# scverse/muon

Measured on AMD Instinct MI355X. Metric: cells/sec for TF-IDF+LSI(k=50), higher is better.
Workload: dtype f32

## Files before the change

include/muon_amd.h:

```cpp
#ifndef MUON_AMD_H
#define MUON_AMD_H

#include <stddef.h>
#include <stdint.h>

#ifdef __cplusplus
extern "C" {
#endif

typedef enum {
  MU_OK = 0,
  MU_ERR_ARG = -1,
  MU_ERR_HIP = -2,
  MU_ERR_NO_DEVICE = -3,
  MU_ERR_UNSUPPORTED = -4
} mu_status;

#define MU_DTYPE_F32 0
#define MU_DTYPE_F64 1

#define MU_TFIDF_LOG_TF 1
#define MU_TFIDF_LOG_IDF 2
#define MU_TFIDF_LOG_TFIDF 4

int mu_version(void);
const char* mu_last_error(void);
int mu_device_count(int* count);
int mu_set_device(int device);
int mu_device_info(int device, char* name, int len, int* n_cu, size_t* total_mem);
int mu_malloc(void** d_ptr, size_t bytes);
int mu_free(void* d_ptr);
int mu_memcpy_h2d(void* d_dst, const void* h_src, size_t bytes, void* stream);
int mu_memcpy_d2h(void* h_dst, const void* d_src, size_t bytes, void* stream);
int mu_memset(void* d_dst, int value, size_t bytes, void* stream);
int mu_stream_sync(void* stream);
int mu_host_hash64(const void* h_ptr, size_t n_bytes, int n_threads, uint64_t seed, uint64_t* h_out);

size_t mu_csr_row_col_sums_worksize(int64_t n_rows, int64_t n_cols);

int mu_csr_row_col_sums(int dtype, int64_t n_rows, int64_t n_cols, const int64_t* d_indptr,
                        const int32_t* d_indices, const void* d_values, double* d_rowsum,
                        double* d_colsum, void* d_work, size_t work_bytes, void* stream);

int mu_tfidf_idf(int dtype, int64_t n_cols, double n_obs, const double* d_colsum, int flags,
                 void* d_idf, void* stream);

int mu_tfidf_scale(int dtype, int64_t n_rows, const int64_t* d_indptr, const int32_t* d_indices,
                   const void* d_values, const double* d_rowsum, const void* d_idf, double scale,
                   int flags, void* d_out, unsigned long long* d_zero_count, void* stream);

int mu_tfidf_scale_sweep(int dtype, int64_t n_rows, int64_t n_cols, const int64_t* d_indptr,
                         const int32_t* d_indices, const void* d_values, const double* d_rowsum,
                         const void* d_idf, double scale, int flags, void* d_out,
                         unsigned long long* d_zero_count, void* d_work, size_t work_bytes,
                         int have_slab_ptr, void* stream);

int mu_csr_count_nonzero(int dtype, int64_t n_rows, const int64_t* d_indptr, const void* d_values,
                         int64_t* d_row_nnz, void* stream);
int mu_csr_compact_nonzero(int dtype, int64_t n_rows, const int64_t* d_indptr,
                           const int32_t* d_indices, const void* d_values,
                           const int64_t* d_new_indptr, int32_t* d_new_indices, void* d_new_values,
                           void* stream);
int mu_exclusive_scan_i64(int64_t n, const int64_t* d_in, int64_t* d_out, void* stream);

int mu_binarize_values(int dtype, int64_t nnz, void* d_values, void* stream);

size_t mu_csr_qc_worksize(int64_t n_rows, int64_t n_cols);
int mu_csr_qc(int dtype, int64_t n_rows, int64_t n_cols, const int64_t* d_indptr, const int32_t* d_indices,
              const void* d_values, int64_t* d_row_nnz, double* d_rowsum, int64_t* d_col_nnz, double* d_colsum,
              void* d_work, size_t work_bytes, const int64_t* d_slab_ptr, void* stream);

int mu_csr_submatrix_count(int64_t n_rows, int64_t n_cols, int64_t n_keep, const int64_t* d_indptr,
                           const int32_t* d_indices, const int64_t* d_rows, const int32_t* d_col_table,
                           int64_t* d_new_row_nnz, void* stream);
int mu_csr_submatrix_fill(int dtype, int64_t n_rows, int64_t n_cols, int64_t n_keep, const int64_t* d_indptr,
                          const int32_t* d_indices, const void* d_values, const int64_t* d_rows,
                          const int32_t* d_col_table, const int64_t* d_new_indptr, int32_t* d_new_indices,
                          void* d_new_values, void* stream);

int mu_frag_chunk(void);
int mu_frag_ranges(int64_t n_win, int64_t n_contigs, const int32_t* d_wchrom, const int32_t* d_wlo,
                   const int32_t* d_whi, const int64_t* d_chrom_ptr, const int32_t* d_start, int64_t max_len,
                   int64_t* d_rng_lo, int64_t* d_rng_len, void* stream);
int mu_frag_overlap_count(int64_t n_win, int64_t n_chunks, const int64_t* d_chunk_ptr, const int64_t* d_rng_lo,
                          const int64_t* d_rng_len, const int32_t* d_wlo, const int32_t* d_whi, const int32_t* d_start,
                          const int32_t* d_end, const int32_t* d_barcode, const int32_t* d_cell_of, int64_t n_barcodes,
                          int64_t n_obs, int64_t* d_chunk_cnt, void* stream);
int mu_frag_overlap_emit(int64_t n_win, int64_t n_chunks, const int64_t* d_chunk_ptr, const int64_t* d_rng_lo,
                         const int64_t* d_rng_len, const int32_t* d_wlo, const int32_t* d_whi, const int32_t* d_start,
                         const int32_t* d_end, const int32_t* d_barcode, const int32_t* d_score,
                         const int32_t* d_cell_of, int64_t n_barcodes, int64_t n_obs, int64_t n_features,
                         const int64_t* d_chunk_off, int64_t* d_keys, int32_t* d_vals, void* stream);
int mu_frag_pileup(int64_t n_win, int64_t n_chunks, const int64_t* d_chunk_ptr, const int64_t* d_rng_lo,
                   const int64_t* d_rng_len, const int32_t* d_wlo, const int32_t* d_whi, const int32_t* d_start,
                   const int32_t* d_end, const int32_t* d_barcode, const int32_t* d_score, const int32_t* d_cell_of,
                   int64_t n_barcodes, int64_t n_obs, int64_t width, int32_t* d_diff, void* stream);
int mu_frag_pileup_scan(int64_t n_obs, int64_t width, int64_t flank_size, int64_t center_dist, int32_t* d_diff,
                        int64_t* d_sums, void* stream);
int mu_frag_length_classes(int64_t n_take, const int32_t* d_start, const int32_t* d_end, const int32_t* d_barcode,
                           const int32_t* d_cell_of, int64_t n_barcodes, int64_t n_obs, int free_bound, int mono_bound,
                           int32_t* d_classes, void* stream);

size_t mu_csr_transpose_worksize(int64_t n_rows, int64_t n_cols, int64_t nnz);
int mu_csr_transpose(int dtype, int64_t n_rows, int64_t n_cols, int64_t nnz,
                     const int64_t* d_indptr, const int32_t* d_indices, const void* d_values,
                     int64_t* d_t_indptr, int32_t* d_t_indices, void* d_t_values, void* d_work,
                     size_t work_bytes, void* stream);

int mu_spmm_f32(int64_t n_rows, int64_t n_cols, const int64_t* d_indptr, const int32_t* d_indices,
                const float* d_values, const float* d_Q, int B, float* d_Y, int accumulate,
                void* stream);


int mu_spmm_stream_k(int64_t n_rows);

int mu_tfidf_scale_sweep_stream(int64_t n_rows, int64_t n_cols, const int64_t* d_indptr, const int32_t* d_indices,
                                const float* d_values, const double* d_rowsum, const float* d_idf, double scale,
                                int flags, float* d_out, unsigned long long* d_zero_count, void* d_work,
                                size_t work_bytes, int have_slab_ptr, const int64_t* d_slab_ptr,
                                const int64_t* d_row_dst, void* d_ent, void* stream);
int mu_csr_slab_ptr(int64_t n_rows, int64_t n_cols, const int64_t* d_indptr, const int32_t* d_indices, int64_t* d_sp,
                    void* stream);
int mu_csr_slab_ptr_width(int64_t n_rows, int64_t n_cols, int64_t width, const int64_t* d_indptr,
                          const int32_t* d_indices, int64_t* d_sp, void* stream);
int mu_csr_row_col_sums_sp(int dtype, int64_t n_rows, int64_t n_cols, const int64_t* d_indptr,
                           const int32_t* d_indices, const void* d_values, double* d_rowsum, double* d_colsum,
                           void* d_work, size_t work_bytes, const int64_t* d_slab_ptr, void* stream);
int mu_tfidf_scale_sweep_sp(int dtype, int64_t n_rows, int64_t n_cols, const int64_t* d_indptr,
                            const int32_t* d_indices, const void* d_values, const double* d_rowsum, const void* d_idf,
                            double scale, int flags, void* d_out, unsigned long long* d_zero_count,
                            const int64_t* d_slab_ptr, void* stream);
int mu_tpack4_supported(int64_t n_rows, int64_t n_cols, int64_t nnz);
int mu_tpack4_geometry(int64_t n_rows, int64_t n_cols, int64_t nnz, int64_t* rows_per_block, int* n_blocks,
                       int* tile_cols);
size_t mu_tpack4_worksize(int64_t n_rows, int64_t n_cols, int64_t nnz);
int mu_tpack4_count(int64_t n_rows, int64_t n_cols, int64_t nnz, const int64_t* d_indptr, const int32_t* d_indices,
                    int64_t* d_col_nnz, void* d_work, size_t work_bytes, const int64_t* d_slab_ptr, void* stream);
int mu_tpack4_fill_stream(int64_t n_rows, int64_t n_cols, int64_t nnz, const int64_t* d_indptr,
                          const int32_t* d_indices, const float* d_values, const int64_t* d_x_row_dst,
                          const void* d_x_ent, const int64_t* d_sptr, const int32_t* d_inv, void* d_ent, void* d_work,
                          size_t work_bytes, void* stream);
int mu_tpack4_fill_csr(int64_t n_rows, int64_t n_cols, int64_t nnz, const int64_t* d_indptr, const int32_t* d_indices,
                       const float* d_values, const int64_t* d_x_row_dst, const void* d_x_ent,
                       const int64_t* d_t_indptr, int32_t* d_t_indices, float* d_t_values, void* d_work,
                       size_t work_bytes, void* stream);
int mu_tpack4_status(const void* d_work, int64_t n_rows, int64_t n_cols, int64_t nnz, int* h_err);
size_t mu_tpack4_err_offset(int64_t n_rows, int64_t n_cols, int64_t nnz);
size_t mu_tpack4_cnt_offset(int64_t n_rows, int64_t n_cols, int64_t nnz);
int mu_tpack4_phase_cycles(unsigned long long* h_out6, int reset);
int mu_tperm_stage_pairs(void);
int mu_tperm_plan(int64_t n_rows, int64_t n_cols, int64_t nnz, const int64_t* d_indptr, const int32_t* d_indices,
                  const int64_t* d_x_row_dst, int tile_cols, const int64_t* d_tile_off, int32_t* d_ntile,
                  int32_t* d_tiles, uint32_t* d_cont, uint16_t* d_slots, void* stream);
int mu_tperm_fill(int64_t n_rows, int64_t n_cols, int64_t nnz, const int64_t* d_indptr, const int64_t* d_x_row_dst,
                  const void* d_x_ent, const int64_t* d_cdst, const void* d_cnt, const int64_t* d_tile_off,
                  const int32_t* d_tiles, const uint32_t* d_cont, const uint16_t* d_slots, void* d_ent, void* stream);
int mu_csr_stream_len(int64_t n_pos, const int32_t* d_perm, const int64_t* d_indptr, int64_t* d_len,
                      void* stream);
int mu_csr_stream_fill(int64_t n_pos, const int32_t* d_perm, const int64_t* d_indptr,
                       const int32_t* d_indices, const float* d_values, const int64_t* d_sptr,
                       void* d_ent, void* stream);
int mu_spmm_stream_f32(int64_t n_pos, int64_t n_cols, const int64_t* d_sptr, const void* d_ent,
                       const int32_t* d_perm, int k_layout, const float* d_Q, int B, float* d_Y,
                       void* stream);
int mu_csr_slice_stream(int n_ranges, const int64_t* h_row0, const int64_t* h_rows, const int64_t* h_lo,
                        const int64_t* h_hi, int64_t n_cols, const int64_t* d_indptr, const int32_t* d_indices,
                        const float* d_values, const int64_t* d_slab_ptr, int64_t* d_sptr, void* d_ent, uint32_t* d_rel,
                        void* stream);
int mu_spmm_stream_ranges_f32(int64_t n_pos, const int64_t* d_sptr, const void* d_ent, const int32_t* d_perm,
                              int k_layout, const float* d_Q, int64_t q_rows, float* d_Y, int64_t y_stride,
                              const uint32_t* d_tbl, int64_t tbl_stride, int n_ranges, const int32_t* h_ranges5,
                              int per_wg, void* stream);
int mu_spmm_stream_f64(int64_t n_pos, int64_t n_cols, const int64_t* d_sptr, const void* d_ent,
                       const int32_t* d_perm, int k_layout, const double* d_Q, int B, double* d_Y,
                       int accumulate, void* stream);
int mu_spmm_stream_slab_ok(int B, int K, int slab_cols);
int mu_spmm_stream_slab_f32(int64_t n_pos, int64_t n_cols, const int64_t* d_sptr, const void* d_ent,
                            const int32_t* d_perm, int k_layout, const float* d_Q, int B, float* d_Y,
                            int slab_cols, void* stream);
int mu_spmm_stream_ranges_slab_f32(int64_t n_pos, const int64_t* d_sptr, const void* d_ent, const int32_t* d_perm,
                                   int k_layout, const float* d_Q, int64_t q_rows, float* d_Y, int64_t y_stride,
                                   const uint32_t* d_tbl, int64_t tbl_stride, int n_ranges, const int32_t* h_ranges5,
                                   int per_wg, int slab_cols, void* stream);


int mu_spmm_ell16_waves(int64_t n_rows);
int mu_spmm_ell16_f32(int waves, int64_t n_pos, int64_t n_cols, const int32_t* d_hdr, const int64_t* d_wave_base,
                      const void* d_ent, const int32_t* d_perm, const float* d_Q, float* d_Y, void* stream);
int mu_spmm_ell16_f64(int waves, int64_t n_pos, int64_t n_cols, const int32_t* d_hdr, const int64_t* d_wave_base,
                      const void* d_ent, const int32_t* d_perm, const double* d_Q, double* d_Y, int accumulate,
                      void* stream);
int mu_spmm_ell16_parts(int64_t n_rows, int64_t n_cols, int wide, int* waves, int* parts);
int mu_spmm_ell16_parts_f32(int waves, int parts, int64_t n_pos, int64_t n_cols, const int32_t* d_hdr,
                            const int64_t* d_wave_base, const void* d_ent, const int32_t* d_perm, const float* d_Q,
                            float* d_Y, int64_t y_stride, void* stream);
int mu_spmm_ell16_parts_f64(int waves, int parts, int64_t n_pos, int64_t n_cols, const int32_t* d_hdr,
                            const int64_t* d_wave_base, const void* d_ent, const int32_t* d_perm, const double* d_Q,
                            double* d_Y, int64_t y_stride, void* stream);

int mu_ell16_fill(int64_t n_groups, int64_t n_cols, int64_t nnz, int slab_cols, const int32_t* d_indices, const float* d_values,
                  const int64_t* d_slab_ptr, const int32_t* d_perm, const int32_t* d_hdr, const int64_t* d_win_base,
                  void* d_ent, void* stream);


int mu_tune_set(const char* key, int value);
int mu_tune_get(const char* key);

int mu_spmm_f64(int64_t n_rows, int64_t n_cols, const int64_t* d_indptr, const int32_t* d_indices,
                const double* d_values, const double* d_Q, int B, double* d_Y, int accumulate,
                void* stream);

size_t mu_gram_worksize(int64_t n_rows, int B);
int mu_gram_f32(int64_t n_rows, int B, const float* d_A, double* d_G, double* d_colsum,
                void* d_work, size_t work_bytes, void* stream);

int mu_gram_cross_f32(int64_t n_rows, int B, const float* d_A, const float* d_Bm, double* d_C,
                      void* d_work, size_t work_bytes, void* stream);

int mu_dense_apply_f32(int64_t n_rows, int B, const float* d_A, const float* d_M,
                       const float* d_bias, float* d_Out, void* stream);
int mu_dense_project_out_f32(int64_t n_rows, int B, const float* d_A, const double* d_C, float* d_Z,
                             void* stream);

int mu_chol_rinv_f64(int B, int w, const double* d_G, float* d_M, int* d_flag, void* stream);

int mu_randn_f32(int64_t count, uint64_t seed, float* d_out, void* stream);

size_t mu_skinny_tn_worksize(int dtype, int64_t n_rows, int64_t D);
int mu_skinny_nn(int dtype, int64_t n_rows, int64_t D, int64_t ldY, const void* d_Y, const void* d_T,
                 void* d_out, void* stream);
int mu_skinny_tn(int dtype, int64_t n_rows, int64_t D, int64_t ldY, const void* d_Y, const void* d_Z,
                 void* d_C, void* d_work, size_t work_bytes, void* stream);
int mu_skinny_nn_f64_f32(int64_t n_rows, int64_t D, int64_t ldY, const float* d_Y, const double* d_T, double* d_out,
                         void* stream);
int mu_skinny_tn_f64_f32(int64_t n_rows, int64_t D, int64_t ldY, const float* d_Y, const double* d_Z, double* d_C,
                         void* d_work, size_t work_bytes, void* stream);

int mu_mofa_update_w(int dtype, int64_t D, int K, int G, const void* d_B, const void* d_tau,
                     const void* d_Gz, const void* d_Z2, const void* d_alpha, const void* d_lth,
                     const void* d_l1mth, int spikeslab, void* d_EW, void* d_EW2, void* d_gamma,
                     void* d_EWh2, void* d_sig2, void* stream);
int mu_mofa_update_z(int dtype, int64_t N, int K, int M, int G, const void* d_A, const void* d_pres,
                     const int32_t* d_grp, const void* d_Gw, const void* d_dw2, const void* d_alphaz,
                     const void* d_corr, void* d_EZ, void* d_EZ2, void* d_sig2, void* stream);

size_t mu_mofa_rowstats_work_doubles(int K);
int mu_mofa_rowstats(int dtype, int64_t r0, int64_t r1, int K, const void* d_E, const void* d_E2,
                     const void* d_wgt, const void* d_aux, int scale_out, void* d_out_pad, int ld, int col0,
                     void* d_out_t, int64_t ld_t, void* d_gram, void* d_s2, void* d_s1, double* d_work,
                     void* stream);

int mu_dense_col_moments_chunks(int64_t n_rows, int64_t D);
int mu_dense_col_moments(int dtype, int64_t r0, int64_t r1, int64_t D, const void* d_Y, int chunks,
                         double* d_partial, void* stream);

int mu_knn_filter_f64(int64_t n_q, int64_t c_lo, int64_t c_hi, int p_pad, const double* d_Xq, const double* d_Xc,
                      const double* d_sqq, const double* d_sqc, const double* d_thr, const int32_t* d_self_pos,
                      int cap, int32_t* d_buf_pos, double* d_buf_d, int32_t* d_cnt, void* stream);
int mu_knn_merge_f64(int64_t n_q, int kc, int cap, const double* d_cur_d, const int64_t* d_cur_p, const double* d_buf_d,
                     const int32_t* d_buf_pos, const int32_t* d_cnt, double* d_out_d, int64_t* d_out_p, double* d_thr,
                     void* stream);

int mu_wnn_bandwidth_f64(int64_t n, int p, const double* d_X, const int64_t* d_g_indptr, const int32_t* d_g_indices,
                         const int64_t* d_r_indptr, const int32_t* d_r_indices, int n_bw, double bbox,
                         double* d_csigma, int32_t* d_overflow, void* stream);

int mu_mofa_gs_update(int dtype, int64_t n, int K, const void* d_T, const void* d_b, const double* d_prior,
                      const double* d_lth, const double* d_l1mth, int spikeslab, void* d_E, void* d_E2,
                      void* d_gamma, void* d_Eh2, void* d_sig2, void* stream);

int mu_umap_strengths_f64(int64_t n, int k, const double* d_dist, const int64_t* d_idx, double target, double mean_all,
                          double* d_val, void* stream);

int mu_csr_densify_rows(int dtype, int64_t r0, int64_t r1, int64_t D, const int64_t* d_indptr,
                        const int32_t* d_indices, const void* d_values, void* d_out, void* stream);

int mu_mofa_jaakkola(int dtype, int64_t n, const void* d_zeta, const void* d_a, const void* d_b, void* d_out,
                     void* stream);

int mu_mofa_poisson_pseudo(int dtype, int64_t n_rows, int64_t D, int mode, const void* d_zeta, const void* d_Y,
                           const void* d_kappa, void* d_out, void* stream);

int64_t mu_mofa_poisson_blocks(int64_t n_own, int64_t n_other);
int64_t mu_mofa_poisson_blocks_for(int dtype, int mode, int K, int64_t n_own, int64_t n_other);
int mu_mofa_poisson_dense(int dtype, int mode, int64_t n_own, int64_t n_other, int K, int64_t other_block,
                          const void* d_E_own, const void* d_E_other, const void* d_kappa, void* d_part, void* stream);
int mu_mofa_poisson_sparse(int dtype, int mode, int64_t n_own, int K, const int64_t* d_indptr, const int32_t* d_indices,
                           const void* d_values, const void* d_E_own, const void* d_E_other, void* d_out, void* stream);
int mu_mofa_poisson_dense_ld(int dtype, int mode, int64_t n_own, int64_t n_other, int K, int ld, int64_t other_block,
                             const void* d_E_own, const void* d_E_other, const void* d_kappa, void* d_part,
                             void* stream);
int mu_mofa_poisson_sparse_ld(int dtype, int mode, int64_t n_own, int K, int ld, const int64_t* d_indptr,
                              const int32_t* d_indices, const void* d_values, const void* d_E_own, const void* d_E_other,
                              void* d_out, void* stream);

int mu_mofa_jaakkola_cols(int K);
int mu_mofa_pack_moments(int dtype, int64_t n, int K, int ldm, const void* d_E, const void* d_E2, void* d_M,
                         void* stream);
int64_t mu_mofa_jaakkola_blocks(int dtype, int K, int64_t n_own, int64_t n_other);
int mu_mofa_jaakkola_sweep(int dtype, int64_t n_own, int64_t n_other, int K, int64_t other_block, const void* d_E_own,
                           const void* d_E2_own, const void* d_E_other, const void* d_E2_other, const void* d_M_other,
                           int ldm, void* d_part, void* stream);

size_t mu_mofa_elbo_work_doubles(int K);
int mu_mofa_tau_elbo(int dtype, int64_t D, int K, int G, const void* d_yy, const void* d_Ngm,
                     const void* d_EW, const void* d_EW2, const void* d_B, const void* d_Gz,
                     const void* d_Z2, double a0, double b0, void* d_tau, void* d_ltau, double* d_elbo,
                     double* d_work, void* stream);
int mu_mofa_stats_resid(int dtype, int64_t D, int K, int64_t q_rows, const double* d_yy, const void* d_EW,
// ... 88 lines not shown
```

muon_amd/csrc/runtime.hip:

```cpp
#include <atomic>
#include <cstdarg>
#include <cstdio>
#include <cstring>
#include <thread>
#include <vector>
#include "common.hpp"

static thread_local char g_err[512] = "";

void mu_set_error(const char* fmt, ...) {
  va_list ap;
  va_start(ap, fmt);
  vsnprintf(g_err, sizeof(g_err), fmt, ap);
  va_end(ap);
}

int mu_num_cus() {
  static int cached[64] = {0};
  int dev = 0;
  if (hipGetDevice(&dev) != hipSuccess || dev < 0 || dev >= 64) return 256;
  if (cached[dev] == 0) {
    int n = 0;
    if (hipDeviceGetAttribute(&n, hipDeviceAttributeMultiprocessorCount, dev) != hipSuccess ||
        n <= 0)
      n = 256;
    cached[dev] = n;
  }
  return cached[dev];
}

static const char* const kTuneKeys[] = {"spmm_k", "spmm_mode", "gram_wg", "pack_wg", "tpack_dbg", "spmm_narrow_off", "ell_mode", "tfidf_wide", "tfidf_pipe", "nn_interleave", "tfidf_abl", "tfidf_sum_m", "tn_pipe", "nn_fast_off", "stream_pipe", "tpack4_m", "tpack4_c", "scale_stream_off", "tpack4_plain", "tpack4_abl", "tpack4_late", "tpack4_circ", "tpack4_off", "tperm_off", "pois_valu", "pois_lane", "spmm_slab"};
constexpr int kTuneN = sizeof(kTuneKeys) / sizeof(kTuneKeys[0]);
static int g_tune[kTuneN] = {};

extern "C" {

int mu_version(void) { return 807; }

int mu_tune_set(const char* key, int value) {
  MU_REQUIRE(key, "null key");
  for (int i = 0; i < kTuneN; ++i)
    if (strcmp(key, kTuneKeys[i]) == 0) {
      MU_REQUIRE(value >= 0, "negative value");
      MU_REQUIRE(i != 0 || value <= 16, "spmm_k must be 0..16");
      g_tune[i] = value;
      return MU_OK;
    }
  mu_set_error("mu_tune_set: unknown key %s", key);
  return MU_ERR_ARG;
}

int mu_tune_get(const char* key) {
  if (key)
    for (int i = 0; i < kTuneN; ++i)
      if (strcmp(key, kTuneKeys[i]) == 0) return g_tune[i];
  return -1;
}

const char* mu_last_error(void) { return g_err; }

int mu_device_count(int* count) {
  MU_REQUIRE(count, "null count");
  int n = 0;
  hipError_t e = hipGetDeviceCount(&n);
  if (e != hipSuccess) {
    *count = 0;
    mu_set_error("hipGetDeviceCount: %s", hipGetErrorString(e));
    return MU_ERR_NO_DEVICE;
  }
  *count = n;
  return MU_OK;
}

int mu_set_device(int device) {
  MU_CHECK_HIP(hipSetDevice(device));
  return MU_OK;
}

int mu_device_info(int device, char* name, int len, int* n_cu, size_t* total_mem) {
  hipDeviceProp_t p;
  MU_CHECK_HIP(hipGetDeviceProperties(&p, device));
  if (name && len > 0) {
    snprintf(name, (size_t)len, "%s (%s)", p.name, p.gcnArchName);
  }
  if (n_cu) *n_cu = p.multiProcessorCount;
  if (total_mem) *total_mem = p.totalGlobalMem;
  return MU_OK;
}

int mu_malloc(void** d_ptr, size_t bytes) {
  MU_REQUIRE(d_ptr, "null out pointer");
  MU_CHECK_HIP(hipMalloc(d_ptr, bytes));
  return MU_OK;
}

int mu_free(void* d_ptr) {
  MU_CHECK_HIP(hipFree(d_ptr));
  return MU_OK;
}

int mu_memcpy_h2d(void* d_dst, const void* h_src, size_t bytes, void* stream) {
  MU_CHECK_HIP(hipMemcpyAsync(d_dst, h_src, bytes, hipMemcpyHostToDevice, (hipStream_t)stream));
  return MU_OK;
}

int mu_memcpy_d2h(void* h_dst, const void* d_src, size_t bytes, void* stream) {
  MU_CHECK_HIP(hipMemcpyAsync(h_dst, d_src, bytes, hipMemcpyDeviceToHost, (hipStream_t)stream));
  return MU_OK;
}

int mu_memset(void* d_dst, int value, size_t bytes, void* stream) {
  MU_CHECK_HIP(hipMemsetAsync(d_dst, value, bytes, (hipStream_t)stream));
  return MU_OK;
}

static inline uint64_t mu_rotl64(uint64_t x, int r) { return (x << r) | (x >> (64 - r)); }
static const uint64_t kP1 = 0x9E3779B185EBCA87ull, kP2 = 0xC2B2AE3D27D4EB4Full, kP3 = 0x165667B19E3779F9ull,
                      kP4 = 0x85EBCA77C2B2AE63ull, kP5 = 0x27D4EB2F165667C5ull;
static inline uint64_t mu_round64(uint64_t acc, uint64_t in) { return mu_rotl64(acc + in * kP2, 31) * kP1; }
static inline uint64_t mu_avalanche64(uint64_t h) {
  h ^= h >> 33; h *= kP2; h ^= h >> 29; h *= kP3; h ^= h >> 32;
  return h;
}
static uint64_t mu_chunk_digest(const unsigned char* p, size_t n, uint64_t seed) {
  uint64_t v1 = seed + kP1 + kP2, v2 = seed + kP2, v3 = seed, v4 = seed - kP1;
  size_t i = 0;
  for (; i + 32 <= n; i += 32) {
    uint64_t w[4];
    memcpy(w, p + i, 32);
    v1 = mu_round64(v1, w[0]); v2 = mu_round64(v2, w[1]); v3 = mu_round64(v3, w[2]); v4 = mu_round64(v4, w[3]);
  }
  uint64_t h = mu_rotl64(v1, 1) + mu_rotl64(v2, 7) + mu_rotl64(v3, 12) + mu_rotl64(v4, 18);
  h = (h ^ mu_round64(0, v1)) * kP1 + kP4; h = (h ^ mu_round64(0, v2)) * kP1 + kP4;
  h = (h ^ mu_round64(0, v3)) * kP1 + kP4; h = (h ^ mu_round64(0, v4)) * kP1 + kP4;
  h += (uint64_t)n;
  for (; i + 8 <= n; i += 8) {
    uint64_t w;
    memcpy(&w, p + i, 8);
    h = mu_rotl64(h ^ mu_round64(0, w), 27) * kP1 + kP4;
  }
  for (; i < n; ++i) h = mu_rotl64(h ^ (p[i] * kP5), 11) * kP1;
  return mu_avalanche64(h);
}

int mu_host_hash64(const void* h_ptr, size_t n_bytes, int n_threads, uint64_t seed, uint64_t* h_out) {
  MU_REQUIRE(h_out && (h_ptr || n_bytes == 0), "null pointer");
  const size_t chunk = (size_t)16 << 20;
  const size_t n_chunks = n_bytes ? (n_bytes + chunk - 1) / chunk : 1;
  std::vector<uint64_t> dig(n_chunks, 0);
  const unsigned char* p = (const unsigned char*)h_ptr;
  std::atomic<size_t> next(0);
  auto work = [&]() {
    for (;;) {
      const size_t c = next.fetch_add(1);
      if (c >= n_chunks) break;
      const size_t lo = c * chunk, hi = (lo + chunk < n_bytes) ? lo + chunk : n_bytes;
      dig[c] = mu_chunk_digest(p + lo, hi - lo, seed + c);
    }
  };
  int T = n_threads < 1 ? 1 : (n_threads > 64 ? 64 : n_threads);
  if ((size_t)T > n_chunks) T = (int)n_chunks;
  std::vector<std::thread> th;
  try {
    if (T > 1) {
      th.reserve(T - 1);
      for (int t = 1; t < T; ++t) th.emplace_back(work);
    }
  } catch (...) {
  }
  work();
  for (auto& x : th) x.join();
  uint64_t h = seed ^ kP5 ^ (uint64_t)n_bytes;
  for (size_t c = 0; c < n_chunks; ++c) h = mu_rotl64(h ^ mu_round64(0, dig[c]), 27) * kP1 + kP4;
  *h_out = mu_avalanche64(h);
  return MU_OK;
}

int mu_stream_sync(void* stream) {
  MU_CHECK_HIP(hipStreamSynchronize((hipStream_t)stream));
  return MU_OK;
}

}
```

muon_amd/csrc/tperm.hip:

```cpp
#include <type_traits>
#include <utility>

#include "common.hpp"
#pragma clang diagnostic ignored "-Winline-asm"

namespace {

constexpr int kT = 1024, kNW = 16;
constexpr int kMaxC = 512;
constexpr int kCap = 9216;
constexpr int kH0 = 72;
constexpr int kW0 = 76;
constexpr int kS0 = 110;
constexpr int kSlotP = 16;
constexpr int kNone = 0xff;

#define MU_TP_CLOB                                                                                                      \
  "v72", "v73", "v74", "v75", "v76", "v77", "v78", "v79", "v80", "v81", "v82", "v83", "v84", "v85", "v86", "v87", "v88", \
      "v89", "v90", "v91", "v92", "v93", "v94", "v95", "v96", "v97", "v98", "v99", "v100", "v101", "v102", "v103",       \
      "v104", "v105", "v106", "v107", "v108", "v109", "v110", "v111", "v112", "v113", "v114", "v115", "v116", "v117",    \
      "v118", "v119", "v120", "v121", "v122", "v123", "v124", "v125", "v126", "v127"

template <int L>
__device__ __forceinline__ int tp_writelane_c(int v, int x) {
// ... 77 lines not shown
      const int ws = wave_sum_all(n);
      if (lane == 0 && ws) atomicAdd(&s_tot, (unsigned)ws);
      __syncthreads();
      total = s_tot;
      __syncthreads();
      if (total <= (unsigned)kCap) break;
      if (tid == 0) s_tot = 0u;
      int w = ((int)(cend - cb) / 2 / 16) * 16;
      w = w < 16 ? 16 : w;
      cend = (int)cb + w;
      __syncthreads();
    }
    if (REC) {
      if (tid == 0) tiles[tb + t] = (int32_t)cb;
      const unsigned over = (unsigned)__ballot(n > 32);
      if (lane == 0) {
        int pa = kNone, pb = kNone;
        if (over) {
          pa = __builtin_ctz(over);
          const unsigned o2 = over & (over - 1u);
          if (o2) pb = __builtin_ctz(o2);
        }
        cont[(tc + t) * kNW + wave] = (uint32_t)(pa | (pb << 8));
      }
      if (total > 0u) {
        const int W = cend - (int)cb;
        for (int k = 0; k < n; ++k) atomicOr(&bm[wave][indices[cur + k] - (int)cb], 1u << sub);
        __syncthreads();
        uint32_t mine = 0;
        if (tid < W)
          for (int w = 0; w < kNW; ++w) mine += (uint32_t)__popc(bm[w][tid]);
        uint32_t incl = mine;
#pragma unroll
        for (int off = 1; off < 64; off <<= 1) {
          const uint32_t u = __shfl_up(incl, off, 64);
          if (lane >= off) incl += u;
        }
        if (lane == 63) wsum[wave] = incl;
        __syncthreads();
        uint32_t run = incl - mine;
        for (int w = 0; w < wave; ++w) run += wsum[w];
        if (tid < W)
          for (int w = 0; w < kNW; ++w) {
            fs[w][tid] = run;
            run += (uint32_t)__popc(bm[w][tid]);
          }
        __syncthreads();
        for (int k = 0; k < n; ++k) {
          const int c = indices[cur + k] - (int)cb;
          slots[dst0 + cur + k] = (uint16_t)(fs[wave][c] + (uint32_t)__popc(bm[wave][c] & ((1u << sub) - 1u)));
        }
        __syncthreads();
        if (tid < W)
          for (int w = 0; w < kNW; ++w) bm[w][tid] = 0u;
      }
    }
    cur += n;
    cb = cend;
  }
  if (tid == 0) {
    if (REC) tiles[tb + t] = (int32_t)n_cols;
    else ntile[g] = t;
  }
}

template <int J>
__device__ __forceinline__ void tp_issue_circ(uint64_t b0, uint64_t b1, uint64_t tb0, uint64_t tb1, unsigned s0, unsigned s1,
                                              unsigned m0, unsigned m1, unsigned sub, unsigned sub8, unsigned sub8w,
                                              unsigned sub2, unsigned sub2w) {
  unsigned long long save;
  unsigned p0, p1, q0, q1;
  asm volatile(
      "s_mov_b64 %[save], exec\n\t"
      "v_cmp_gt_u32 vcc, %[s0], %[sub]\n\t"
      "v_cndmask_b32 %[p0], %[sub8], %[sub8w], vcc\n\t"
      "v_cndmask_b32 %[q0], %[sub2], %[sub2w], vcc\n\t"
      "v_cmp_gt_u32 vcc, %[s1], %[sub]\n\t"
      "v_cndmask_b32 %[p1], %[sub8], %[sub8w], vcc\n\t"
      "v_cndmask_b32 %[q1], %[sub2], %[sub2w], vcc\n\t"
      "s_mov_b32 exec_lo, %[m0]\n\t"
      "s_mov_b32 exec_hi, 0\n\t"
      "global_load_dwordx2 v[%c[C]:%c[V]], %[p0], %[b0]\n\t"
      "global_load_ushort v%c[S], %[q0], %[tb0]\n\t"
      "s_mov_b32 exec_lo, 0\n\t"
      "s_mov_b32 exec_hi, %[m1]\n\t"
      "global_load_dwordx2 v[%c[C]:%c[V]], %[p1], %[b1]\n\t"
      "global_load_ushort v%c[S], %[q1], %[tb1]\n\t"
      "s_mov_b64 exec, %[save]"
      : [save] "=&s"(save), [p0] "=&v"(p0), [p1] "=&v"(p1), [q0] "=&v"(q0), [q1] "=&v"(q1)
      : [sub] "v"(sub), [sub8] "v"(sub8), [sub8w] "v"(sub8w), [sub2] "v"(sub2), [sub2w] "v"(sub2w), [b0] "s"(b0),
        [b1] "s"(b1), [tb0] "s"(tb0), [tb1] "s"(tb1), [s0] "s"(s0), [s1] "s"(s1), [m0] "s"(m0), [m1] "s"(m1),
        [C] "i"(kW0 + 2 * J), [V] "i"(kW0 + 2 * J + 1), [S] "i"(kS0 + J)
      : MU_TP_CLOB, "vcc", "memory");
}
__device__ __forceinline__ void tp_issue_cont(uint64_t a0, uint64_t a1, uint64_t t0, uint64_t t1, int n0, int n1,
                                              unsigned sub8, unsigned sub2) {
  unsigned long long save, m0, m1;
  asm volatile(
      "s_bfm_b64 %[m0], %[n0], 0\n\t"
      "s_bfm_b64 %[m1], %[n1], 32\n\t"
      "s_mov_b64 %[save], exec\n\t"
      "v_mov_b32 v%c[C], 0x7fffffff\n\t"
      "s_mov_b64 exec, %[m0]\n\t"
      "global_load_dwordx2 v[%c[C]:%c[V]], %[o8], %[a0]\n\t"
      "global_load_ushort v%c[S], %[o2], %[t0]\n\t"
      "s_mov_b64 exec, %[m1]\n\t"
      "global_load_dwordx2 v[%c[C]:%c[V]], %[o8], %[a1]\n\t"
      "global_load_ushort v%c[S], %[o2], %[t1]\n\t"
      "s_mov_b64 exec, %[save]"
      : [save] "=&s"(save), [m0] "=&s"(m0), [m1] "=&s"(m1)
      : [o8] "v"(sub8), [o2] "v"(sub2), [a0] "s"(a0), [a1] "s"(a1), [t0] "s"(t0), [t1] "s"(t1), [n0] "s"(n0), [n1] "s"(n1),
        [C] "i"(kW0 + 2 * kSlotP), [V] "i"(kW0 + 2 * kSlotP + 1), [S] "i"(kS0 + kSlotP)
      : MU_TP_CLOB, "memory");
}
template <int J>
__device__ __forceinline__ void tp_pad_slot() {
  asm volatile("v_mov_b32 v%c0, 0x7fffffff" ::"i"(kW0 + 2 * J) : MU_TP_CLOB);
}
template <int J>
__device__ __forceinline__ void tp_retire_slot(int cend, int pad) {
  asm volatile(
      "v_cmp_le_i32 vcc, %0, v%c1\n\t"
      "v_cndmask_b32 v%c1, %2, v%c1, vcc" ::"s"(cend),
      "i"(kW0 + 2 * J), "v"(pad)
      : MU_TP_CLOB, "vcc");
}
__device__ __forceinline__ void tp_wait_all() { asm volatile("s_waitcnt vmcnt(0)" ::: MU_TP_CLOB, "memory"); }
template <int R>
__device__ __forceinline__ unsigned tp_reg() {
  unsigned v;
  asm volatile("v_mov_b32 %0, v%c1" : "=v"(v) : "i"(R) : MU_TP_CLOB);
  return v;
}
__device__ __forceinline__ void tp_issue_header(const uint32_t* bg, const uint32_t* bn, const int64_t* cd, unsigned off4) {
  asm volatile(
      "global_load_dword v%c4, %0, %1\n\t"
      "global_load_dword v%c5, %0, %2\n\t"
      "v_lshlrev_b32 v%c6, 1, %0\n\t"
      "global_load_dwordx2 v[%c6:%c7], v%c6, %3"
      :
      : "v"(off4), "s"(bg), "s"(bn), "s"(cd), "i"(kH0), "i"(kH0 + 1), "i"(kH0 + 2), "i"(kH0 + 3)
      : MU_TP_CLOB, "memory");
}

template <int... I, class F>
__device__ __forceinline__ void tp_for_impl(std::integer_sequence<int, I...>, F&& f) {
  (f(std::integral_constant<int, I>{}), ...);
}
template <int N, class F>
__device__ __forceinline__ void tp_for(F&& f) {
  tp_for_impl(std::make_integer_sequence<int, N>{}, static_cast<F&&>(f));
}

__global__ __launch_bounds__(kT) __attribute__((amdgpu_num_vgpr(36))) void k_tperm_move(
    int64_t n_rows, int64_t n_cols, int rw, int G, const int64_t* __restrict__ indptr,
    const int64_t* __restrict__ row_dst, const unsigned long long* __restrict__ xent,
    const int64_t* __restrict__ cdst, const uint32_t* __restrict__ base, const int64_t* __restrict__ toff,
    const int32_t* __restrict__ tiles, const uint32_t* __restrict__ cont, const uint16_t* __restrict__ slots,
    unsigned long long* __restrict__ out) {
  __shared__ unsigned long long stage[2][kCap];
  __shared__ uint32_t lrun[2][kMaxC];
  __shared__ int64_t gdst[2][kMaxC];
  __shared__ uint32_t wsum[2][kNW];
  int g = blockIdx.x;
  if (G > 0) {
    const int per = (G + 7) / 8;
    g = (g % 8) * per + (g / 8);
    if (g >= G) return;
  } else {
    G = -G;
  }
  const int tid = threadIdx.x, lane = tid & 63;
  const int wave = uniform32(tid >> 6);
  const int half = lane >> 5, sub = lane & 31;
  const int64_t rpb = (int64_t)kNW * rw;
  const int64_t r0 = (int64_t)g * rpb;
  const int64_t r1 = (r0 + rpb) < n_rows ? (r0 + rpb) : n_rows;
  const int64_t wr0 = r0 + (int64_t)wave * rw;

  uint64_t A = 0;
  int rem = 0, ld = 0;
  {
    const int64_t row = wr0 + sub;
    const bool ok = sub < rw && row < r1;
    const int64_t p0 = ok ? indptr[row] : 0;
    rem = ok ? (int)(indptr[row + 1] - p0) : 0;
    A = (uint64_t)xent + 8ull * (uint64_t)(ok ? row_dst[row] : 0);
  }
  const int64_t tb = uniform64(toff[g]) + g;
  const int nt = (int)(uniform64(toff[g + 1]) - uniform64(toff[g]));
  const uint32_t* cw = cont + (tb - g) * kNW + wave;
  const unsigned subo = (unsigned)sub * 8u, sub2 = (unsigned)sub * 2u;
  tp_for<16>([&](auto jc) { tp_pad_slot<decltype(jc)::value>(); });

  auto cont_of = [&](int t) { return t < nt ? uniform32((int)cw[(int64_t)t * kNW]) : (kNone | (kNone << 8)); };
  auto issue_all = [&](int pw) {
    const int remc = rem < 32 ? rem : 32;
    const int nn = remc - ld;
    const uint64_t st = A + 8ull * (uint64_t)(unsigned)ld;
    const unsigned s5 = (unsigned)(st >> 3) & 31u;
    const unsigned rot = __builtin_rotateleft32((unsigned)((1ull << nn) - 1ull), s5);
    const uint64_t b256 = st & ~255ull;
    const uint64_t tb64 = (uint64_t)slots + ((b256 - (uint64_t)xent) >> 2);
    ld = remc;
    tp_for<16>([&](auto jc) {
      constexpr int J = decltype(jc)::value;
      tp_issue_circ<J>(tp_readlane_u64(b256, 2 * J), tp_readlane_u64(b256, 2 * J + 1), tp_readlane_u64(tb64, 2 * J),
                       tp_readlane_u64(tb64, 2 * J + 1), (unsigned)__builtin_amdgcn_readlane((int)s5, 2 * J),
                       (unsigned)__builtin_amdgcn_readlane((int)s5, 2 * J + 1),
                       (unsigned)__builtin_amdgcn_readlane((int)rot, 2 * J),
                       (unsigned)__builtin_amdgcn_readlane((int)rot, 2 * J + 1), (unsigned)sub, subo, subo + 256u, sub2,
                       sub2 + 64u);
    });
    const int pa = pw & 0xff, pb = pw >> 8;
    if (pa != kNone) {
      const int lb = pb != kNone ? pb : pa;
      int na = __builtin_amdgcn_readlane(rem, pa) - 32, nb = pb != kNone ? __builtin_amdgcn_readlane(rem, pb) - 32 : 0;
      na = __builtin_amdgcn_readfirstlane(na < 0 ? 0 : (na > 32 ? 32 : na));
      nb = __builtin_amdgcn_readfirstlane(nb < 0 ? 0 : (nb > 32 ? 32 : nb));
      const uint64_t a0 = tp_readlane_u64(A, pa) + 256u, a1 = tp_readlane_u64(A, lb) + 256u;
      tp_issue_cont(a0, a1, (uint64_t)slots + ((a0 - (uint64_t)xent) >> 2), (uint64_t)slots + ((a1 - (uint64_t)xent) >> 2),
                    na, nb, subo, sub2);
    }
  };
  const uint32_t* base_g = base + (int64_t)g * n_cols;
  const uint32_t* base_n = base + (int64_t)(g + 1) * n_cols;
  auto issue_header = [&](int64_t cb) {
    int64_t ofs = n_cols - 1 - cb;
    if (ofs < 0) {
      ofs = 0;
      cb = n_cols - 1;
    }
    const unsigned o4 = (unsigned)((int64_t)tid < ofs ? (int64_t)tid : ofs) * 4u;
    tp_issue_header(base_g + cb, base_n + cb, cdst + cb, o4);
  };
  uint32_t mine = 0, incl = 0;
  int64_t gd = 0;
  auto take_header = [&](int W, int set) {
    const uint32_t b0 = tp_reg<kH0>(), b1 = tp_reg<kH0 + 1>();
    const unsigned lo = tp_reg<kH0 + 2>(), hi = tp_reg<kH0 + 3>();
    mine = tid < W ? b1 - b0 : 0u;
    gd = (int64_t)(((unsigned long long)hi << 32) | lo) + (int64_t)b0;
    incl = mine;
#pragma unroll
    for (int off = 1; off < 64; off <<= 1) {
      const uint32_t u = __shfl_up(incl, off, 64);
      if (lane >= off) incl += u;
    }
    if (lane == 63) wsum[set][wave] = incl;
  };
  auto finish_header = [&](int W, int set) {
    uint32_t wpre = 0;
#pragma unroll
    for (int w = 0; w < kNW; ++w) {
      const uint32_t u = wsum[set][w];
      if (w < wave) wpre += u;
    }
    if (tid < W) {
      lrun[set][tid] = (mine << 16) | (wpre + incl - mine);
      gdst[set][tid] = gd;
    }
  };
  auto write_out = [&](int set, int ncol) {
    const unsigned long long* stg = stage[set];
    const int grp = tid >> 4, s16 = tid & 15;
    for (int c0 = grp; c0 < ncol; c0 += 4 * (kT / 16)) {
      uint32_t lr[4];
      int64_t gq[4];
      unsigned long long e[4];
#pragma unroll
      for (int u = 0; u < 4; ++u) {
        const int cl = c0 + u * (kT / 16);
        const bool in = cl < ncol;
        lr[u] = in ? lrun[set][in ? cl : 0] : 0u;
        gq[u] = gdst[set][in ? cl : 0];
      }
#pragma unroll
      for (int u = 0; u < 4; ++u) {
        const uint32_t L = lr[u] >> 16, src = lr[u] & 0xffffu;
        e[u] = stg[(uint32_t)s16 < L ? src + s16 : 0];
      }
#pragma unroll
      for (int u = 0; u < 4; ++u) {
        const uint32_t L = lr[u] >> 16, src = lr[u] & 0xffffu;
        if ((uint32_t)s16 < L) out[gq[u] + s16] = e[u];
        for (uint32_t i = 16 + s16; i < L; i += 16) out[gq[u] + i] = stg[src + i];
      }
    }
  };

  auto tile_at = [&](int t) { return uniform32(tiles[tb + (t < nt ? t : nt)]); };
  int c0 = tile_at(0), c1 = tile_at(1), c2 = tile_at(2);
  issue_header(c0);
  tp_wait_all();
  take_header(c1 - c0, 0);
  int pw = cont_of(0);
  issue_all(pw);
  issue_header(c1);
  __syncthreads();
  finish_header(c1 - c0, 0);

  for (int t = 0; t < nt; ++t) {
    const int set = t & 1;
    const int cend = c1;
    int hf = half;
    asm volatile("" : "+v"(hf));
    const int pw_next = cont_of(t + 1);
    tp_wait_all();
    take_header(c2 - c1, set ^ 1);
    unsigned long long* stg = stage[set];
    int cntv = 0;
    tp_for<16>([&](auto jc) {
      constexpr int J = decltype(jc)::value;
      const int c = (int)tp_reg<kW0 + 2 * J>();
      const unsigned v = tp_reg<kW0 + 2 * J + 1>(), s = tp_reg<kS0 + J>();
      const bool valid = c < cend;
      const unsigned long long m = __ballot(valid);
      if (valid) stg[s] = (unsigned long long)(unsigned)(wr0 + 2 * J + hf) | ((unsigned long long)v << 32);
      cntv = tp_writelane_c<2 * J>(cntv, __popc((unsigned)m));
      cntv = tp_writelane_c<2 * J + 1>(cntv, __popc((unsigned)(m >> 32)));
    });
    const int pa = pw & 0xff, pb = pw >> 8;
    if (pa != kNone) {
      const int lb = pb != kNone ? pb : pa;
      const int c = (int)tp_reg<kW0 + 2 * kSlotP>();
      const unsigned v = tp_reg<kW0 + 2 * kSlotP + 1>(), s = tp_reg<kS0 + kSlotP>();
      const bool valid = c < cend;
      const unsigned long long m = __ballot(valid);
      if (valid) stg[s] = (unsigned long long)(unsigned)(wr0 + (hf ? lb : pa)) | ((unsigned long long)v << 32);
      cntv = tp_writelane_s(cntv, __builtin_amdgcn_readlane(cntv, pa) + __popc((unsigned)m), pa);
      if (pb != kNone) cntv = tp_writelane_s(cntv, __builtin_amdgcn_readlane(cntv, pb) + __popc((unsigned)(m >> 32)), pb);
    }
    {
      int padv = 0x7fffffff;
      asm volatile("" : "+v"(padv));
      tp_for<16>([&](auto jc) { tp_retire_slot<decltype(jc)::value>(cend, padv); });
    }
    if (half == 0) {
      A += (uint64_t)(unsigned)cntv * 8u;
      rem -= cntv;
      ld = ld > cntv ? ld - cntv : 0;
    }
    pw = pw_next;
    issue_all(pw);
    issue_header(c2);
    const int c3 = tile_at(t + 3);
    __syncthreads();
    finish_header(c2 - c1, set ^ 1);
    write_out(set, c1 - c0);
    c0 = c1;
    c1 = c2;
    c2 = c3;
  }
  tp_wait_all();
}

}

extern "C" {

int mu_tperm_stage_pairs(void) { return kCap; }

int mu_tperm_plan(int64_t n_rows, int64_t n_cols, int64_t nnz, const int64_t* d_indptr, const int32_t* d_indices,
                  const int64_t* d_x_row_dst, int tile_cols, const int64_t* d_tile_off, int32_t* d_ntile,
                  int32_t* d_tiles, uint32_t* d_cont, uint16_t* d_slots, void* stream) {
  MU_REQUIRE(mu_tpack4_supported(n_rows, n_cols, nnz), "shape out of range (mu_tpack4_supported)");
  MU_REQUIRE(d_indptr && d_indices, "null pointer");
  MU_REQUIRE(tile_cols >= 16 && tile_cols <= kMaxC, "tile_cols out of range (16 .. 512)");
  MU_REQUIRE(d_tile_off ? (d_x_row_dst && d_tiles && d_cont && d_slots) : d_ntile != nullptr,
             "count pass: d_ntile; record pass: d_x_row_dst, d_tile_off, d_tiles, d_cont, d_slots");
  int64_t rpb = 0;
  int G = 0;
  mu_tpack4_geometry(n_rows, n_cols, nnz, &rpb, &G, nullptr);
  const int rw = (int)(rpb / kNW);
  hipStream_t st = (hipStream_t)stream;
  if (d_tile_off)
    hipLaunchKernelGGL((k_tperm_plan<true>), dim3(G), dim3(kT), 0, st, n_rows, n_cols, tile_cols, rw, d_indptr, d_indices,
                       d_x_row_dst, d_tile_off, d_ntile, d_tiles, d_cont, d_slots);
  else
    hipLaunchKernelGGL((k_tperm_plan<false>), dim3(G), dim3(kT), 0, st, n_rows, n_cols, tile_cols, rw, d_indptr,
                       d_indices, d_x_row_dst, d_tile_off, d_ntile, d_tiles, d_cont, d_slots);
  MU_CHECK_LAUNCH();
  return MU_OK;
}

int mu_tperm_fill(int64_t n_rows, int64_t n_cols, int64_t nnz, const int64_t* d_indptr, const int64_t* d_x_row_dst,
                  const void* d_x_ent, const int64_t* d_cdst, const void* d_cnt, const int64_t* d_tile_off,
                  const int32_t* d_tiles, const uint32_t* d_cont, const uint16_t* d_slots, void* d_ent, void* stream) {
  MU_REQUIRE(mu_tpack4_supported(n_rows, n_cols, nnz), "shape out of range (mu_tpack4_supported)");
  MU_REQUIRE(d_indptr && d_x_row_dst && d_x_ent && d_cdst && d_cnt && d_tile_off && d_tiles && d_cont && d_slots && d_ent,
             "null pointer");
  MU_REQUIRE((reinterpret_cast<uintptr_t>(d_x_ent) & 255) == 0, "the row stream of X must be 256-byte aligned");
  int64_t rpb = 0;
  int G = 0;
  mu_tpack4_geometry(n_rows, n_cols, nnz, &rpb, &G, nullptr);
  const int rw = (int)(rpb / kNW);
  const bool xcd = mu_tune_get("tpack4_plain") != 1;
  const unsigned grid = xcd ? (unsigned)(8 * ((G + 7) / 8)) : (unsigned)G;
  hipLaunchKernelGGL(k_tperm_move, dim3(grid), dim3(kT), 0, (hipStream_t)stream, n_rows, n_cols, rw, xcd ? G : -G,
                     d_indptr, d_x_row_dst, (const unsigned long long*)d_x_ent, d_cdst, (const uint32_t*)d_cnt, d_tile_off,
                     d_tiles, d_cont, d_slots, (unsigned long long*)d_ent);
  MU_CHECK_LAUNCH();
  return MU_OK;
}

}
```

Baseline: 3.710 million.

## Encode column index in staged entries and flatten tperm write-out loop

The staged entry now carries its local column id in the low word, and the per-column shared tables (run length and destination) collapse into a single per-column destination offset table. The write-out loop changes from per-column groups of 16 lanes, which idle on short columns, to flat strided rounds over all staged entries, each looking up its destination offset. A vectorised wave-sum prefix also produces the tile total. A templated variant that records per-phase cycle counts is added for profiling, but it is not used by default.

```diff
diff --git a/include/muon_amd.h b/include/muon_amd.h
--- a/include/muon_amd.h
+++ b/include/muon_amd.h
@@ -155,6 +155,10 @@
 int mu_tperm_fill(int64_t n_rows, int64_t n_cols, int64_t nnz, const int64_t* d_indptr, const int64_t* d_x_row_dst,
                   const void* d_x_ent, const int64_t* d_cdst, const void* d_cnt, const int64_t* d_tile_off,
                   const int32_t* d_tiles, const uint32_t* d_cont, const uint16_t* d_slots, void* d_ent, void* stream);
+int mu_tperm_fill_phases(int64_t n_rows, int64_t n_cols, int64_t nnz, const int64_t* d_indptr,
+                         const int64_t* d_x_row_dst, const void* d_x_ent, const int64_t* d_cdst, const void* d_cnt,
+                         const int64_t* d_tile_off, const int32_t* d_tiles, const uint32_t* d_cont,
+                         const uint16_t* d_slots, void* d_ent, unsigned long long* d_phases, void* stream);
 int mu_csr_stream_len(int64_t n_pos, const int32_t* d_perm, const int64_t* d_indptr, int64_t* d_len,
                       void* stream);
 int mu_csr_stream_fill(int64_t n_pos, const int32_t* d_perm, const int64_t* d_indptr,
diff --git a/muon_amd/csrc/runtime.hip b/muon_amd/csrc/runtime.hip
--- a/muon_amd/csrc/runtime.hip
+++ b/muon_amd/csrc/runtime.hip
@@ -35,7 +35,7 @@
 
 extern "C" {
 
-int mu_version(void) { return 807; }
+int mu_version(void) { return 808; }
 
 int mu_tune_set(const char* key, int value) {
   MU_REQUIRE(key, "null key");
diff --git a/muon_amd/csrc/tperm.hip b/muon_amd/csrc/tperm.hip
--- a/muon_amd/csrc/tperm.hip
+++ b/muon_amd/csrc/tperm.hip
@@ -253,16 +253,17 @@
   tp_for_impl(std::make_integer_sequence<int, N>{}, static_cast<F&&>(f));
 }
 
-__global__ __launch_bounds__(kT) __attribute__((amdgpu_num_vgpr(36))) void k_tperm_move(
+constexpr int kPhases = 6;
+template <bool ACCT>
+__device__ __forceinline__ void tperm_move_body(
     int64_t n_rows, int64_t n_cols, int rw, int G, const int64_t* __restrict__ indptr,
     const int64_t* __restrict__ row_dst, const unsigned long long* __restrict__ xent,
     const int64_t* __restrict__ cdst, const uint32_t* __restrict__ base, const int64_t* __restrict__ toff,
     const int32_t* __restrict__ tiles, const uint32_t* __restrict__ cont, const uint16_t* __restrict__ slots,
-    unsigned long long* __restrict__ out) {
+    unsigned long long* __restrict__ out, unsigned long long* __restrict__ acct) {
   __shared__ unsigned long long stage[2][kCap];
-  __shared__ uint32_t lrun[2][kMaxC];
-  __shared__ int64_t gdst[2][kMaxC];
-  __shared__ uint32_t wsum[2][kNW];
+  __shared__ int64_t dcol[2][kMaxC];
+  __shared__ __attribute__((aligned(16))) uint32_t wsum[2][kNW];
   int g = blockIdx.x;
   if (G > 0) {
     const int per = (G + 7) / 8;
@@ -351,43 +352,49 @@
     if (lane == 63) wsum[set][wave] = incl;
   };
   auto finish_header = [&](int W, int set) {
-    uint32_t wpre = 0;
-#pragma unroll
-    for (int w = 0; w < kNW; ++w) {
-      const uint32_t u = wsum[set][w];
-      if (w < wave) wpre += u;
-    }
-    if (tid < W) {
-      lrun[set][tid] = (mine << 16) | (wpre + incl - mine);
-      gdst[set][tid] = gd;
-    }
+    const uint4* ws4 = reinterpret_cast<const uint4*>(wsum[set]);
+    uint32_t wpre = 0, total = 0;
+#pragma unroll
+    for (int q = 0; q < kNW / 4; ++q) {
+      const uint4 u4 = ws4[q];
+      const uint32_t u[4] = {u4.x, u4.y, u4.z, u4.w};
+#pragma unroll
+      for (int k = 0; k < 4; ++k) {
+        total += u[k];
+        wpre += u[k] & (uint32_t)-(int)(4 * q + k < wave);
+      }
+    }
+    if (tid < W) dcol[set][tid] = gd - (int64_t)(wpre + incl - mine);
+    return uniform32((int)total);
   };
-  auto write_out = [&](int set, int ncol) {
+  auto write_out = [&](int set, int total) {
     const unsigned long long* stg = stage[set];
-    const int grp = tid >> 4, s16 = tid & 15;
-    for (int c0 = grp; c0 < ncol; c0 += 4 * (kT / 16)) {
-      uint32_t lr[4];
-      int64_t gq[4];
-      unsigned long long e[4];
-#pragma unroll
-      for (int u = 0; u < 4; ++u) {
-        const int cl = c0 + u * (kT / 16);
-        const bool in = cl < ncol;
-        lr[u] = in ? lrun[set][in ? cl : 0] : 0u;
-        gq[u] = gdst[set][in ? cl : 0];
-      }
-#pragma unroll
-      for (int u = 0; u < 4; ++u) {
-        const uint32_t L = lr[u] >> 16, src = lr[u] & 0xffffu;
-        e[u] = stg[(uint32_t)s16 < L ? src + s16 : 0];
-      }
-#pragma unroll
-      for (int u = 0; u < 4; ++u) {
-        const uint32_t L = lr[u] >> 16, src = lr[u] & 0xffffu;
-        if ((uint32_t)s16 < L) out[gq[u] + s16] = e[u];
-        for (uint32_t i = 16 + s16; i < L; i += 16) out[gq[u] + i] = stg[src + i];
-      }
-    }
+    const int64_t* dc = dcol[set];
+    auto rounds = [&](auto nc, int i) {
+      constexpr int N = decltype(nc)::value;
+      unsigned long long e[N];
+      int64_t q[N];
+#pragma unroll
+      for (int u = 0; u < N; ++u) e[u] = stg[i + u * kT];
+#pragma unroll
+      for (int u = 0; u < N; ++u) q[u] = dc[((unsigned)e[u] >> 16) & (unsigned)(kMaxC - 1)];
+#pragma unroll
+      for (int u = 0; u < N; ++u)
+        out[q[u] + (i + u * kT)] =
+            (e[u] & 0xffffffff00000000ull) | (unsigned long long)((unsigned)r0 + ((unsigned)e[u] & 0xffffu));
+    };
+    const int whole = total / kT;
+    int r = 0;
+    for (; r + 4 <= whole; r += 4) rounds(std::integral_constant<int, 4>{}, tid + r * kT);
+    if ((whole - r) & 2) {
+      rounds(std::integral_constant<int, 2>{}, tid + r * kT);
+      r += 2;
+    }
+    if ((whole - r) & 1) {
+      rounds(std::integral_constant<int, 1>{}, tid + r * kT);
+      r += 1;
+    }
+    if (tid + r * kT < total) rounds(std::integral_constant<int, 1>{}, tid + r * kT);
   };
 
   auto tile_at = [&](int t) { return uniform32(tiles[tb + (t < nt ? t : nt)]); };
@@ -399,7 +406,18 @@
   issue_all(pw);
   issue_header(c1);
   __syncthreads();
-  finish_header(c1 - c0, 0);
+  int tot = finish_header(c1 - c0, 0);
+
+  unsigned long long ph[kPhases] = {}, t_prev = 0;
+  if constexpr (ACCT) t_prev = __builtin_amdgcn_s_memtime();
+  auto stamp = [&](auto kc) {
+    if constexpr (ACCT) {
+      const unsigned long long now = __builtin_amdgcn_s_memtime();
+      ph[decltype(kc)::value] += now - t_prev;
+      t_prev = now;
+    }
+  };
+  using std::integral_constant;
 
   for (int t = 0; t < nt; ++t) {
     const int set = t & 1;
@@ -408,8 +426,11 @@
     asm volatile("" : "+v"(hf));
     const int pw_next = cont_of(t + 1);
     tp_wait_all();
+    stamp(integral_constant<int, 0>{});
     take_header(c2 - c1, set ^ 1);
+    stamp(integral_constant<int, 1>{});
     unsigned long long* stg = stage[set];
+    const unsigned wbase = (unsigned)(wave * rw) - ((unsigned)c0 << 16);
     int cntv = 0;
     tp_for<16>([&](auto jc) {
       constexpr int J = decltype(jc)::value;
@@ -417,7 +438,7 @@
       const unsigned v = tp_reg<kW0 + 2 * J + 1>(), s = tp_reg<kS0 + J>();
       const bool valid = c < cend;
       const unsigned long long m = __ballot(valid);
-      if (valid) stg[s] = (unsigned long long)(unsigned)(wr0 + 2 * J + hf) | ((unsigned long long)v << 32);
+      if (valid) stg[s] = (unsigned long long)(((unsigned)c << 16) + (wbase + 2 * J + hf)) | ((unsigned long long)v << 32);
       cntv = tp_writelane_c<2 * J>(cntv, __popc((unsigned)m));
       cntv = tp_writelane_c<2 * J + 1>(cntv, __popc((unsigned)(m >> 32)));
     });
@@ -428,10 +449,11 @@
       const unsigned v = tp_reg<kW0 + 2 * kSlotP + 1>(), s = tp_reg<kS0 + kSlotP>();
       const bool valid = c < cend;
       const unsigned long long m = __ballot(valid);
-      if (valid) stg[s] = (unsigned long long)(unsigned)(wr0 + (hf ? lb : pa)) | ((unsigned long long)v << 32);
+      if (valid) stg[s] = (unsigned long long)(((unsigned)c << 16) + (wbase + (hf ? lb : pa))) | ((unsigned long long)v << 32);
       cntv = tp_writelane_s(cntv, __builtin_amdgcn_readlane(cntv, pa) + __popc((unsigned)m), pa);
       if (pb != kNone) cntv = tp_writelane_s(cntv, __builtin_amdgcn_readlane(cntv, pb) + __popc((unsigned)(m >> 32)), pb);
     }
+    stamp(integral_constant<int, 2>{});
     {
       int padv = 0x7fffffff;
       asm volatile("" : "+v"(padv));
@@ -446,14 +468,44 @@
     issue_all(pw);
     issue_header(c2);
     const int c3 = tile_at(t + 3);
+    stamp(integral_constant<int, 3>{});
     __syncthreads();
-    finish_header(c2 - c1, set ^ 1);
-    write_out(set, c1 - c0);
+    stamp(integral_constant<int, 4>{});
+    const int tot_next = finish_header(c2 - c1, set ^ 1);
+    write_out(set, tot);
+    tot = tot_next;
+    stamp(integral_constant<int, 5>{});
     c0 = c1;
     c1 = c2;
     c2 = c3;
   }
   tp_wait_all();
+  if constexpr (ACCT) {
+    if (lane == 0) {
+      unsigned long long* row = acct + ((int64_t)g * kNW + wave) * (kPhases + 2);
+#pragma unroll
+      for (int k = 0; k < kPhases; ++k) row[k] = ph[k];
+      row[kPhases] = (unsigned long long)nt;
+      row[kPhases + 1] = 0ull;
+    }
+  }
+}
+
+__global__ __launch_bounds__(kT) __attribute__((amdgpu_num_vgpr(36))) void k_tperm_move(
+    int64_t n_rows, int64_t n_cols, int rw, int G, const int64_t* __restrict__ indptr,
+    const int64_t* __restrict__ row_dst, const unsigned long long* __restrict__ xent,
+    const int64_t* __restrict__ cdst, const uint32_t* __restrict__ base, const int64_t* __restrict__ toff,
+    const int32_t* __restrict__ tiles, const uint32_t* __restrict__ cont, const uint16_t* __restrict__ slots,
+    unsigned long long* __restrict__ out) {
+  tperm_move_body<false>(n_rows, n_cols, rw, G, indptr, row_dst, xent, cdst, base, toff, tiles, cont, slots, out, nullptr);
+}
+__global__ __launch_bounds__(kT) __attribute__((amdgpu_num_vgpr(36))) void k_tperm_phases(
+    int64_t n_rows, int64_t n_cols, int rw, int G, const int64_t* __restrict__ indptr,
+    const int64_t* __restrict__ row_dst, const unsigned long long* __restrict__ xent,
+    const int64_t* __restrict__ cdst, const uint32_t* __restrict__ base, const int64_t* __restrict__ toff,
+    const int32_t* __restrict__ tiles, const uint32_t* __restrict__ cont, const uint16_t* __restrict__ slots,
+    unsigned long long* __restrict__ out, unsigned long long* __restrict__ acct) {
+  tperm_move_body<true>(n_rows, n_cols, rw, G, indptr, row_dst, xent, cdst, base, toff, tiles, cont, slots, out, acct);
 }
 
 }
@@ -485,9 +537,10 @@
   return MU_OK;
 }
 
-int mu_tperm_fill(int64_t n_rows, int64_t n_cols, int64_t nnz, const int64_t* d_indptr, const int64_t* d_x_row_dst,
-                  const void* d_x_ent, const int64_t* d_cdst, const void* d_cnt, const int64_t* d_tile_off,
-                  const int32_t* d_tiles, const uint32_t* d_cont, const uint16_t* d_slots, void* d_ent, void* stream) {
+static int tperm_fill(int64_t n_rows, int64_t n_cols, int64_t nnz, const int64_t* d_indptr, const int64_t* d_x_row_dst,
+                      const void* d_x_ent, const int64_t* d_cdst, const void* d_cnt, const int64_t* d_tile_off,
+                      const int32_t* d_tiles, const uint32_t* d_cont, const uint16_t* d_slots, void* d_ent,
+                      unsigned long long* d_phases, void* stream) {
   MU_REQUIRE(mu_tpack4_supported(n_rows, n_cols, nnz), "shape out of range (mu_tpack4_supported)");
   MU_REQUIRE(d_indptr && d_x_row_dst && d_x_ent && d_cdst && d_cnt && d_tile_off && d_tiles && d_cont && d_slots && d_ent,
              "null pointer");
@@ -498,11 +551,32 @@
   const int rw = (int)(rpb / kNW);
   const bool xcd = mu_tune_get("tpack4_plain") != 1;
   const unsigned grid = xcd ? (unsigned)(8 * ((G + 7) / 8)) : (unsigned)G;
-  hipLaunchKernelGGL(k_tperm_move, dim3(grid), dim3(kT), 0, (hipStream_t)stream, n_rows, n_cols, rw, xcd ? G : -G,
-                     d_indptr, d_x_row_dst, (const unsigned long long*)d_x_ent, d_cdst, (const uint32_t*)d_cnt, d_tile_off,
-                     d_tiles, d_cont, d_slots, (unsigned long long*)d_ent);
+  if (d_phases)
+    hipLaunchKernelGGL(k_tperm_phases, dim3(grid), dim3(kT), 0, (hipStream_t)stream, n_rows, n_cols, rw, xcd ? G : -G,
+                       d_indptr, d_x_row_dst, (const unsigned long long*)d_x_ent, d_cdst, (const uint32_t*)d_cnt,
+                       d_tile_off, d_tiles, d_cont, d_slots, (unsigned long long*)d_ent, d_phases);
+  else
+    hipLaunchKernelGGL(k_tperm_move, dim3(grid), dim3(kT), 0, (hipStream_t)stream, n_rows, n_cols, rw, xcd ? G : -G,
+                       d_indptr, d_x_row_dst, (const unsigned long long*)d_x_ent, d_cdst, (const uint32_t*)d_cnt,
+                       d_tile_off, d_tiles, d_cont, d_slots, (unsigned long long*)d_ent);
   MU_CHECK_LAUNCH();
   return MU_OK;
 }
 
-}
+int mu_tperm_fill(int64_t n_rows, int64_t n_cols, int64_t nnz, const int64_t* d_indptr, const int64_t* d_x_row_dst,
+                  const void* d_x_ent, const int64_t* d_cdst, const void* d_cnt, const int64_t* d_tile_off,
+                  const int32_t* d_tiles, const uint32_t* d_cont, const uint16_t* d_slots, void* d_ent, void* stream) {
+  return tperm_fill(n_rows, n_cols, nnz, d_indptr, d_x_row_dst, d_x_ent, d_cdst, d_cnt, d_tile_off, d_tiles, d_cont,
+                    d_slots, d_ent, nullptr, stream);
+}
+
+int mu_tperm_fill_phases(int64_t n_rows, int64_t n_cols, int64_t nnz, const int64_t* d_indptr,
+                         const int64_t* d_x_row_dst, const void* d_x_ent, const int64_t* d_cdst, const void* d_cnt,
+                         const int64_t* d_tile_off, const int32_t* d_tiles, const uint32_t* d_cont,
+                         const uint16_t* d_slots, void* d_ent, unsigned long long* d_phases, void* stream) {
+  MU_REQUIRE(d_phases, "null pointer");
+  return tperm_fill(n_rows, n_cols, nnz, d_indptr, d_x_row_dst, d_x_ent, d_cdst, d_cnt, d_tile_off, d_tiles, d_cont,
+                    d_slots, d_ent, d_phases, stream);
+}
+
+}
```

New measurement: 3.769 million (median of 6 runs). 1.6% higher.
